# CurvineIO/curvine

Measured on AMD Instinct MI355X. Metric: cached_seq_read_GiBps, higher is better.
Workload: dtype bytes; 1 GPU; seqread; model=curvine-amd cache engine, tier=HBM, read_chunk=4194304, threads=32, iodepth=64, block_size=268435456, fuse_channels=8, short_circuit=True, parallelism=shard-per-gpu x1

## Files before the change

csrc/module.cpp:

```cpp

#include <pybind11/pybind11.h>
#include <pybind11/stl.h>

#include <sys/mman.h>

#include <atomic>
#include <cstring>
#include <mutex>
#include <stdexcept>
#include <string>
#include <vector>

#include <hip/hip_runtime.h>

namespace py = pybind11;

#define HIP_CHECK(expr)                                                        \
  do {                                                                         \
    hipError_t _e = (expr);                                                    \
    if (_e != hipSuccess)                                                      \
      throw std::runtime_error(std::string(#expr) + ": " +                     \
                               hipGetErrorString(_e));                         \
  } while (0)


static uint32_t crc_tab[8][256];
static uint32_t comb_mat[24][32];
static const uint32_t CRC_POLY = 0x82F63B78u;
static const int CRC_SUB = 4096;
static const int WG = 256;

static void gf2_square(uint32_t dst[32], const uint32_t src[32]) {
  for (int i = 0; i < 32; ++i) {
    uint32_t v = src[i], out = 0;
    for (int b = 0; b < 32; ++b)
      if ((v >> b) & 1) out ^= src[b];
    dst[i] = out;
  }
}

static uint32_t gf2_apply(const uint32_t mat[32], uint32_t crc) {
  uint32_t out = 0;
  for (int i = 0; i < 32; ++i)
    if ((crc >> i) & 1) out ^= mat[i];
  return out;
}

static void crc_init_tables() {
  for (uint32_t i = 0; i < 256; ++i) {
    uint32_t c = i;
    for (int k = 0; k < 8; ++k) c = (c >> 1) ^ ((c & 1) ? CRC_POLY : 0);
    crc_tab[0][i] = c;
  }
  for (int t = 1; t < 8; ++t)
    for (uint32_t i = 0; i < 256; ++i)
      crc_tab[t][i] = (crc_tab[t - 1][i] >> 8) ^ crc_tab[0][crc_tab[t - 1][i] & 0xFF];

  uint32_t m[32], tmp[32];
  m[0] = CRC_POLY;
  for (int i = 1; i < 32; ++i) m[i] = 1u << (i - 1);
  int shift_bits_log2 = 0;
  {
    uint64_t bits = 8ull * CRC_SUB;
    while ((1ull << shift_bits_log2) < bits) shift_bits_log2++;
  }
  for (int s = 0; s < shift_bits_log2; ++s) {
    gf2_square(tmp, m);
    std::memcpy(m, tmp, sizeof(m));
  }
  std::memcpy(comb_mat[0], m, sizeof(m));
  for (int k = 1; k < 24; ++k) gf2_square(comb_mat[k], comb_mat[k - 1]);
}

static uint32_t crc32c_sw(const uint8_t* p, size_t n, uint32_t crc_in) {
  uint32_t crc = crc_in ^ 0xFFFFFFFFu;
  while (n && ((uintptr_t)p & 7)) { crc = (crc >> 8) ^ crc_tab[0][(crc ^ *p++) & 0xFF]; --n; }
#if defined(__SSE4_2__)
  while (n >= 8) {
    crc = (uint32_t)__builtin_ia32_crc32di(crc, *(const uint64_t*)p);
    p += 8; n -= 8;
  }
  while (n) { crc = __builtin_ia32_crc32qi(crc, *p++); --n; }
#else
  while (n >= 8) {
    uint64_t v = *(const uint64_t*)p;
    uint32_t lo = (uint32_t)v ^ crc, hi = (uint32_t)(v >> 32);
    crc = crc_tab[7][lo & 0xFF] ^ crc_tab[6][(lo >> 8) & 0xFF] ^
          crc_tab[5][(lo >> 16) & 0xFF] ^ crc_tab[4][lo >> 24] ^
          crc_tab[3][hi & 0xFF] ^ crc_tab[2][(hi >> 8) & 0xFF] ^
          crc_tab[1][(hi >> 16) & 0xFF] ^ crc_tab[0][hi >> 24];
    p += 8; n -= 8;
  }
  while (n) { crc = (crc >> 8) ^ crc_tab[0][(crc ^ *p++) & 0xFF]; --n; }
#endif
  return crc ^ 0xFFFFFFFFu;
}

static uint32_t crc32c_shift(uint32_t crc, uint64_t len) {
  if (!len) return crc;
  uint32_t m[32], sq[32];
  m[0] = CRC_POLY;
  for (int i = 1; i < 32; ++i) m[i] = 1u << (i - 1);
  uint64_t bits = 8ull * len;
  while (bits) {
    if (bits & 1) crc = gf2_apply(m, crc);
    bits >>= 1;
    if (bits) { gf2_square(sq, m); std::memcpy(m, sq, sizeof(m)); }
  }
  return crc;
}

static uint32_t crc32c_combine(uint32_t crc1, uint32_t crc2, uint64_t len2) {
  return crc32c_shift(crc1, len2) ^ crc2;
}

#include "kernels.hip"
#include "lz4.hip"


static int cached_device_count = -2;
static int device_count() {
  if (cached_device_count == -2) {
    int n = 0;
    if (hipGetDeviceCount(&n) != hipSuccess) n = 0;
    cached_device_count = n;
  }
  return cached_device_count;
}


#define SPOOL 16

struct Arena {
  void* base = nullptr;
  size_t cap = 0;
  int device = -1;
  bool pinned = false;
  hipStream_t stream = nullptr;
  hipStream_t kstream = nullptr;
  hipStream_t spool[SPOOL] = {};
  std::mutex spool_mu[SPOOL];
  std::atomic<uint32_t> srr{0};
  std::vector<void*> pin;
  std::vector<hipEvent_t> ev;
  size_t pin_sz = 0;
  void* scratch = nullptr;
  size_t scratch_sz = 0;
  bool crc_tables_uploaded = false;
  bool ipc_imported = false;
  std::mutex mu;

  bool is_dev() const { return device >= 0; }
};

static std::vector<Arena*> g_arenas;
static std::mutex g_arenas_mu;

static Arena* get_arena(int h) {
  std::lock_guard<std::mutex> g(g_arenas_mu);
  if (h < 0 || h >= (int)g_arenas.size() || !g_arenas[h])
    throw std::runtime_error("bad arena handle");
  return g_arenas[h];
}

static int arena_create(int device, size_t cap, size_t staging_bytes,
                        int staging_count, bool host_pinned) {
  auto* a = new Arena();
  a->device = device;
  a->cap = cap;
  if (device >= 0) {
    if (device >= device_count()) {
      delete a;
      throw std::runtime_error("no such GPU device");
    }
    HIP_CHECK(hipSetDevice(device));
    HIP_CHECK(hipMalloc(&a->base, cap));
    HIP_CHECK(hipStreamCreateWithFlags(&a->stream, hipStreamNonBlocking));
    HIP_CHECK(hipStreamCreateWithFlags(&a->kstream, hipStreamNonBlocking));
    for (int i = 0; i < SPOOL; ++i)
      HIP_CHECK(hipStreamCreateWithFlags(&a->spool[i], hipStreamNonBlocking));
    a->pin_sz = staging_bytes;
    a->pin.resize(staging_count);
    a->ev.resize(staging_count);
    for (int i = 0; i < staging_count; ++i) {
      HIP_CHECK(hipHostMalloc(&a->pin[i], staging_bytes, hipHostMallocDefault));
      HIP_CHECK(hipEventCreateWithFlags(&a->ev[i], hipEventDisableTiming));
    }
  } else {
    if (host_pinned && device_count() > 0) {
      HIP_CHECK(hipHostMalloc(&a->base, cap, hipHostMallocDefault));
      a->pinned = true;
    } else {
      size_t aligned = (cap + ((2u << 20) - 1)) & ~size_t((2u << 20) - 1);
      if (posix_memalign(&a->base, 2u << 20, aligned) != 0) {
        delete a;
        throw std::bad_alloc();
      }
#ifdef MADV_HUGEPAGE
      madvise(a->base, aligned, MADV_HUGEPAGE);
#endif
      std::memset(a->base, 0, cap);
    }
  }
  std::lock_guard<std::mutex> g(g_arenas_mu);
  for (size_t i = 0; i < g_arenas.size(); ++i)
    if (!g_arenas[i]) { g_arenas[i] = a; return (int)i; }
  g_arenas.push_back(a);
  return (int)g_arenas.size() - 1;
}

static void arena_destroy(int h) {
  Arena* a;
  {
    std::lock_guard<std::mutex> g(g_arenas_mu);
    if (h < 0 || h >= (int)g_arenas.size() || !g_arenas[h]) return;
    a = g_arenas[h];
    g_arenas[h] = nullptr;
  }
  if (a->is_dev()) {
    hipSetDevice(a->device);
    hipStreamSynchronize(a->stream);
    for (auto* p : a->pin) hipHostFree(p);
    for (auto e : a->ev) hipEventDestroy(e);
    if (a->scratch) hipFree(a->scratch);
    if (a->ipc_imported) hipIpcCloseMemHandle(a->base);
    else hipFree(a->base);
    hipStreamDestroy(a->stream);
    hipStreamDestroy(a->kstream);
    for (int i = 0; i < SPOOL; ++i)
      if (a->spool[i]) hipStreamDestroy(a->spool[i]);
  } else if (a->pinned) {
    hipHostFree(a->base);
  } else {
    std::free(a->base);
  }
  delete a;
}


static py::bytes arena_ipc_handle(int h) {
  Arena* a = get_arena(h);
  if (!a->is_dev())
    throw std::runtime_error("ipc export: device arenas only");
  hipIpcMemHandle_t ih;
  HIP_CHECK(hipSetDevice(a->device));
  HIP_CHECK(hipIpcGetMemHandle(&ih, a->base));
  return py::bytes((const char*)&ih, sizeof(ih));
}

static int arena_ipc_open(py::bytes handle, size_t cap, int device) {
  std::string hb = handle;
  if (hb.size() != sizeof(hipIpcMemHandle_t))
    throw std::runtime_error("ipc open: bad handle size");
  if (device < 0 || device >= device_count())
    throw std::runtime_error("ipc open: bad device");
  hipIpcMemHandle_t ih;
  std::memcpy(&ih, hb.data(), sizeof(ih));
  auto* a = new Arena();
  a->device = device;
  a->cap = cap;
  a->ipc_imported = true;
  HIP_CHECK(hipSetDevice(device));
  hipError_t e = hipIpcOpenMemHandle(&a->base, ih,
                                     hipIpcMemLazyEnablePeerAccess);
  if (e != hipSuccess) {
    delete a;
    throw std::runtime_error(std::string("hipIpcOpenMemHandle: ") +
                             hipGetErrorString(e));
  }
  HIP_CHECK(hipStreamCreateWithFlags(&a->stream, hipStreamNonBlocking));
  HIP_CHECK(hipStreamCreateWithFlags(&a->kstream, hipStreamNonBlocking));
  for (int i = 0; i < SPOOL; ++i)
    HIP_CHECK(hipStreamCreateWithFlags(&a->spool[i], hipStreamNonBlocking));
  std::lock_guard<std::mutex> g(g_arenas_mu);
  for (size_t i = 0; i < g_arenas.size(); ++i)
    if (!g_arenas[i]) { g_arenas[i] = a; return (int)i; }
  g_arenas.push_back(a);
  return (int)g_arenas.size() - 1;
}

static void ensure_scratch(Arena* a, size_t n) {
  if (a->scratch_sz >= n) return;
  if (a->scratch) HIP_CHECK(hipFree(a->scratch));
  HIP_CHECK(hipMalloc(&a->scratch, n));
  a->scratch_sz = n;
}

static void ensure_crc_tables(Arena* a) {
  if (a->crc_tables_uploaded) return;
  crc_init_tables();
  HIP_CHECK(hipMemcpyToSymbol(HIP_SYMBOL(g_crc_tab), crc_tab, sizeof(crc_tab)));
  HIP_CHECK(hipMemcpyToSymbol(HIP_SYMBOL(g_comb_mat), comb_mat, sizeof(comb_mat)));
  a->crc_tables_uploaded = true;
}


static void check_range(Arena* a, uint64_t off, uint64_t n) {
  if (off + n > a->cap) throw std::runtime_error("arena range out of bounds");
}

static bool is_pinned_host(const void* p) {
  hipPointerAttribute_t at;
  if (hipPointerGetAttributes(&at, p) != hipSuccess) {
    (void)hipGetLastError();
    return false;
  }
  return at.type == hipMemoryTypeHost;
}

static const uint64_t RING_THRESHOLD = 2u << 20;


struct BouncePair {
  void* pin[2] = {nullptr, nullptr};
  hipEvent_t ev[2] = {};
  int device = -1;
};

static constexpr size_t kBounceSz = 8 << 20;

struct BouncePool {
  std::mutex mu;
  std::unordered_map<int, std::vector<BouncePair*>> free_by_dev;
};
static BouncePool g_bounce;

static BouncePair* bounce_acquire(int device) {
  {
    std::lock_guard<std::mutex> g(g_bounce.mu);
    auto& v = g_bounce.free_by_dev[device];
    if (!v.empty()) {
      BouncePair* b = v.back();
      v.pop_back();
      return b;
    }
  }
  auto* b = new BouncePair();
  b->device = device;
  HIP_CHECK(hipSetDevice(device));
  HIP_CHECK(hipHostMalloc(&b->pin[0], kBounceSz, hipHostMallocDefault));
  HIP_CHECK(hipHostMalloc(&b->pin[1], kBounceSz, hipHostMallocDefault));
  HIP_CHECK(hipEventCreateWithFlags(&b->ev[0], hipEventDisableTiming));
  HIP_CHECK(hipEventCreateWithFlags(&b->ev[1], hipEventDisableTiming));
  return b;
}

static void bounce_release(BouncePair* b) {
  std::lock_guard<std::mutex> g(g_bounce.mu);
  auto& v = g_bounce.free_by_dev[b->device];
  if (v.size() >= 32) {
    hipEventDestroy(b->ev[0]);
    hipEventDestroy(b->ev[1]);
    hipHostFree(b->pin[0]);
    hipHostFree(b->pin[1]);
    delete b;
    return;
  }
  v.push_back(b);
}

static std::atomic<bool> g_process_exiting{false};
static struct ExitFlagSetter {
  ~ExitFlagSetter() { g_process_exiting.store(true); }
} g_exit_flag_setter;

struct TlsStreams {
  hipStream_t s[64] = {};
  ~TlsStreams() {
    if (g_process_exiting.load()) return;
    for (auto x : s)
      if (x) (void)hipStreamDestroy(x);
  }
};

static hipStream_t thread_stream(int device) {
  thread_local TlsStreams tls;
  if (device < 0 || device >= 64) throw std::runtime_error("bad device");
  if (!tls.s[device]) {
    HIP_CHECK(hipSetDevice(device));
    HIP_CHECK(hipStreamCreateWithFlags(&tls.s[device], hipStreamNonBlocking));
  }
  return tls.s[device];
}

static void dev_read_direct(Arena* a, uint64_t off, uint8_t* dst, uint64_t n) {
  HIP_CHECK(hipSetDevice(a->device));
  hipStream_t s = thread_stream(a->device);
  HIP_CHECK(hipMemcpyAsync(dst, (const uint8_t*)a->base + off, n,
                           hipMemcpyDeviceToHost, s));
  HIP_CHECK(hipStreamSynchronize(s));
}

static void dev_write_direct(Arena* a, uint64_t off, const uint8_t* src,
                             uint64_t n) {
  HIP_CHECK(hipSetDevice(a->device));
  hipStream_t s = thread_stream(a->device);
  HIP_CHECK(hipMemcpyAsync((uint8_t*)a->base + off, src, n,
                           hipMemcpyHostToDevice, s));
  HIP_CHECK(hipStreamSynchronize(s));
}

static void dev_read(Arena* a, uint64_t off, uint8_t* dst, uint64_t n) {
  if (n <= RING_THRESHOLD || is_pinned_host(dst)) {
    dev_read_direct(a, off, dst, n);
    return;
  }
  HIP_CHECK(hipSetDevice(a->device));
  BouncePair* bp = bounce_acquire(a->device);
  hipStream_t s = thread_stream(a->device);
  const uint8_t* src = (const uint8_t*)a->base + off;
  uint64_t cs = std::min<uint64_t>(kBounceSz,
                                   std::max<uint64_t>(1u << 20, (n + 1) / 2));
  uint64_t nchunks = (n + cs - 1) / cs;
  try {
    for (uint64_t c = 0; c < nchunks; ++c) {
      uint64_t coff = c * cs;
      uint64_t clen = std::min<uint64_t>(cs, n - coff);
      int slot = (int)(c & 1);
      HIP_CHECK(hipMemcpyAsync(bp->pin[slot], src + coff, clen,
                               hipMemcpyDeviceToHost, s));
      HIP_CHECK(hipEventRecord(bp->ev[slot], s));
      if (c > 0) {
        int prev = (int)((c - 1) & 1);
        HIP_CHECK(hipEventSynchronize(bp->ev[prev]));
        uint64_t poff = (c - 1) * cs;
        std::memcpy(dst + poff, bp->pin[prev],
                    std::min<uint64_t>(cs, n - poff));
      }
    }
    int last = (int)((nchunks - 1) & 1);
    HIP_CHECK(hipEventSynchronize(bp->ev[last]));
    uint64_t loff = (nchunks - 1) * cs;
    std::memcpy(dst + loff, bp->pin[last],
                std::min<uint64_t>(cs, n - loff));
  } catch (...) {
    (void)hipStreamSynchronize(s);
    bounce_release(bp);
    throw;
  }
  bounce_release(bp);
}

static void dev_write(Arena* a, uint64_t off, const uint8_t* src, uint64_t n) {
  if (n <= RING_THRESHOLD || is_pinned_host(src)) {
    dev_write_direct(a, off, src, n);
    return;
  }
  HIP_CHECK(hipSetDevice(a->device));
  BouncePair* bp = bounce_acquire(a->device);
  hipStream_t s = thread_stream(a->device);
  uint8_t* dst = (uint8_t*)a->base + off;
  uint64_t cs = std::min<uint64_t>(kBounceSz,
                                   std::max<uint64_t>(1u << 20, (n + 1) / 2));
  uint64_t nchunks = (n + cs - 1) / cs;
  try {
    for (uint64_t c = 0; c < nchunks; ++c) {
      uint64_t coff = c * cs;
      uint64_t clen = std::min<uint64_t>(cs, n - coff);
      int slot = (int)(c & 1);
      if (c >= 2) HIP_CHECK(hipEventSynchronize(bp->ev[slot]));
      std::memcpy(bp->pin[slot], src + coff, clen);
      HIP_CHECK(hipMemcpyAsync(dst + coff, bp->pin[slot], clen,
                               hipMemcpyHostToDevice, s));
// ... 262 lines not shown
        uint64_t doff = d2 * a->pin_sz;
        std::memcpy(dst + doff, a->pin[ds],
                    std::min<uint64_t>(a->pin_sz, total - doff));
      }
    }
  }
}

static void arena_gather_ptr(
    int h, std::vector<std::tuple<uint64_t, uint64_t, uint64_t>> ext,
    uintptr_t dst_ptr) {
  Arena* a = get_arena(h);
  for (auto& e : ext) check_range(a, std::get<0>(e), std::get<2>(e));
  uint8_t* dst = (uint8_t*)dst_ptr;
  py::gil_scoped_release rel;
  if (!a->is_dev()) {
    for (auto& e : ext)
      std::memcpy(dst + std::get<1>(e), (uint8_t*)a->base + std::get<0>(e),
                  std::get<2>(e));
    return;
  }
  std::lock_guard<std::mutex> g(a->mu);
  HIP_CHECK(hipSetDevice(a->device));
  std::vector<Extent> exts(ext.size());
  std::vector<uint32_t> tile_ext;
  std::vector<uint64_t> tile_off;
  for (size_t i = 0; i < ext.size(); ++i) {
    exts[i] = {std::get<0>(ext[i]), std::get<1>(ext[i]), std::get<2>(ext[i])};
    for (uint64_t t = 0; t < exts[i].len; t += TILE) {
      tile_ext.push_back((uint32_t)i);
      tile_off.push_back(t);
    }
  }
  size_t meta = exts.size() * sizeof(Extent) +
                tile_ext.size() * (sizeof(uint32_t) + sizeof(uint64_t)) + 64;
  ensure_scratch(a, meta);
  Extent* d_ext = (Extent*)a->scratch;
  uint32_t* d_te = (uint32_t*)(d_ext + exts.size());
  uint64_t* d_to = (uint64_t*)(((uintptr_t)(d_te + tile_ext.size()) + 7) & ~7ull);
  HIP_CHECK(hipMemcpyAsync(d_ext, exts.data(), exts.size() * sizeof(Extent),
                           hipMemcpyHostToDevice, a->kstream));
  HIP_CHECK(hipMemcpyAsync(d_te, tile_ext.data(),
                           tile_ext.size() * sizeof(uint32_t),
                           hipMemcpyHostToDevice, a->kstream));
  HIP_CHECK(hipMemcpyAsync(d_to, tile_off.data(),
                           tile_off.size() * sizeof(uint64_t),
                           hipMemcpyHostToDevice, a->kstream));
  int grid = (int)std::min<size_t>(tile_ext.size(), 8192);
  (void)hipGetLastError();
  hipLaunchKernelGGL(copy_extents_kernel, dim3(grid), dim3(WG), 0, a->kstream,
                     (const uint8_t*)a->base, dst, d_ext, d_te, d_to,
                     (uint32_t)tile_ext.size());
  HIP_CHECK(hipGetLastError());
  HIP_CHECK(hipStreamSynchronize(a->kstream));
}

static uintptr_t arena_base_ptr(int h) {
  return (uintptr_t)get_arena(h)->base;
}

static void arena_read_batch(int h, const std::vector<uint64_t>& offs,
                             const std::vector<uint64_t>& dsts, uint64_t n) {
  Arena* a = get_arena(h);
  if (offs.size() != dsts.size())
    throw std::runtime_error("arena_read_batch: offs/dsts mismatch");
  for (uint64_t off : offs) check_range(a, off, n);
  py::gil_scoped_release rel;
  if (!a->is_dev()) {
    for (size_t i = 0; i < offs.size(); ++i)
      std::memcpy((uint8_t*)dsts[i], (uint8_t*)a->base + offs[i], n);
    return;
  }
  HIP_CHECK(hipSetDevice(a->device));
  hipStream_t s = thread_stream(a->device);
  for (size_t i = 0; i < offs.size(); ++i)
    HIP_CHECK(hipMemcpyAsync((void*)dsts[i], (uint8_t*)a->base + offs[i], n,
                             hipMemcpyDeviceToHost, s));
  HIP_CHECK(hipStreamSynchronize(s));
}


struct RdExt { uint64_t file_off, len; int arena; uint64_t arena_off; };
struct RdReader { uint64_t length; std::vector<RdExt> exts; };
static std::mutex g_rd_mu;
static std::unordered_map<int64_t, RdReader> g_rd;
static int64_t g_rd_next = 1;

static int64_t reader_register(
    std::vector<std::tuple<uint64_t, uint64_t, int, uint64_t>> exts,
    uint64_t length) {
  RdReader r;
  r.length = length;
  r.exts.reserve(exts.size());
  uint64_t prev = 0;
  for (auto& e : exts) {
    if (std::get<0>(e) < prev)
      throw std::runtime_error("reader_register: extents must be sorted");
    prev = std::get<0>(e);
    get_arena(std::get<2>(e));
    r.exts.push_back({std::get<0>(e), std::get<1>(e), std::get<2>(e),
                      std::get<3>(e)});
  }
  std::lock_guard<std::mutex> g(g_rd_mu);
  int64_t rid = g_rd_next++;
  g_rd[rid] = std::move(r);
  return rid;
}

static void reader_unregister(int64_t rid) {
  std::lock_guard<std::mutex> g(g_rd_mu);
  g_rd.erase(rid);
}

static py::list reader_pread_batch(int64_t rid,
                                   const std::vector<uint64_t>& offs,
                                   uint64_t n, uintptr_t dst_ptr,
                                   uint64_t stride) {
  RdReader* r;
  {
    std::lock_guard<std::mutex> g(g_rd_mu);
    auto it = g_rd.find(rid);
    if (it == g_rd.end()) throw std::runtime_error("bad reader id");
    r = &it->second;
  }
  std::vector<uint32_t> skipped;
  {
    py::gil_scoped_release rel;
    int used_dev[8];
    int n_dev = 0;
    const auto& exts = r->exts;
    for (size_t i = 0; i < offs.size(); ++i) {
      uint64_t off = offs[i];
      const RdExt* e = nullptr;
      if (off + n <= r->length && !exts.empty()) {
        size_t lo = 0, hi = exts.size();
        while (lo < hi) {
          size_t mid = (lo + hi) / 2;
          if (exts[mid].file_off <= off) lo = mid + 1; else hi = mid;
        }
        if (lo > 0 && off - exts[lo - 1].file_off + n <= exts[lo - 1].len)
          e = &exts[lo - 1];
      }
      if (e == nullptr) {
        skipped.push_back((uint32_t)i);
        continue;
      }
      uint64_t boff = off - e->file_off;
      Arena* a = get_arena(e->arena);
      uint8_t* dst = (uint8_t*)dst_ptr + i * stride;
      const uint8_t* src = (uint8_t*)a->base + e->arena_off + boff;
      if (!a->is_dev()) {
        std::memcpy(dst, src, n);
      } else {
        HIP_CHECK(hipSetDevice(a->device));
        HIP_CHECK(hipMemcpyAsync(dst, src, n, hipMemcpyDeviceToHost,
                                 thread_stream(a->device)));
        bool seen = false;
        for (int d = 0; d < n_dev; d++) seen |= (used_dev[d] == a->device);
        if (!seen && n_dev < 8) used_dev[n_dev++] = a->device;
      }
    }
    for (int d = 0; d < n_dev; d++) {
      HIP_CHECK(hipSetDevice(used_dev[d]));
      HIP_CHECK(hipStreamSynchronize(thread_stream(used_dev[d])));
    }
  }
  py::list out;
  for (uint32_t i : skipped) out.append(i);
  return out;
}


static py::bytes lz4_compress_py(py::buffer buf) {
  py::buffer_info info = buf.request(false);
  const uint8_t* src = (const uint8_t*)info.ptr;
  size_t n = (size_t)info.size * info.itemsize;
  uint32_t n_chunks = (uint32_t)((n + LZ4_CHUNK - 1) / LZ4_CHUNK);
  std::vector<uint32_t> sizes(n_chunks);
  std::vector<uint8_t> out;
  out.reserve(n / 2 + 1024);
  size_t header = 4 + 8 + 4 + 4 + 4ull * n_chunks;
  out.resize(header);
  {
    py::gil_scoped_release rel;
    std::vector<uint8_t> tmp(LZ4_CHUNK + LZ4_CHUNK / 128 + 64);
    for (uint32_t c = 0; c < n_chunks; ++c) {
      size_t cn = std::min<size_t>(LZ4_CHUNK, n - (size_t)c * LZ4_CHUNK);
      size_t cs = lz4_compress_block(src + (size_t)c * LZ4_CHUNK, cn,
                                     tmp.data());
      sizes[c] = (uint32_t)cs;
      out.insert(out.end(), tmp.data(), tmp.data() + cs);
    }
    uint8_t* h = out.data();
    memcpy(h, &LZ4_MAGIC, 4);
    uint64_t raw = n;
    memcpy(h + 4, &raw, 8);
    uint32_t ck = LZ4_CHUNK;
    memcpy(h + 12, &ck, 4);
    memcpy(h + 16, &n_chunks, 4);
    memcpy(h + 20, sizes.data(), 4ull * n_chunks);
  }
  return py::bytes((const char*)out.data(), out.size());
}

struct Lz4Header {
  uint64_t raw_size;
  uint32_t chunk_size, n_chunks;
  const uint32_t* sizes;
  const uint8_t* payload;
};

static Lz4Header lz4_parse(const uint8_t* p, size_t n) {
  if (n < 20) throw std::runtime_error("lz4: short container");
  uint32_t magic;
  memcpy(&magic, p, 4);
  if (magic != LZ4_MAGIC) throw std::runtime_error("lz4: bad magic");
  Lz4Header h;
  memcpy(&h.raw_size, p + 4, 8);
  memcpy(&h.chunk_size, p + 12, 4);
  memcpy(&h.n_chunks, p + 16, 4);
  if (n < 20 + 4ull * h.n_chunks) throw std::runtime_error("lz4: truncated");
  h.sizes = (const uint32_t*)(p + 20);
  h.payload = p + 20 + 4ull * h.n_chunks;
  uint64_t payload_n = 0;
  for (uint32_t c = 0; c < h.n_chunks; ++c) payload_n += h.sizes[c];
  if (payload_n > n - 20 - 4ull * h.n_chunks)
    throw std::runtime_error("lz4: truncated");
  if ((uint64_t)h.n_chunks * h.chunk_size < h.raw_size ||
      (h.n_chunks && (uint64_t)(h.n_chunks - 1) * h.chunk_size >= h.raw_size))
    throw std::runtime_error("lz4: chunk table does not match raw size");
  return h;
}

static py::bytes lz4_decompress_py(py::buffer buf) {
  py::buffer_info info = buf.request(false);
  const uint8_t* src = (const uint8_t*)info.ptr;
  size_t n = (size_t)info.size * info.itemsize;
  Lz4Header h = lz4_parse(src, n);
  std::string out(h.raw_size, '\0');
  {
    py::gil_scoped_release rel;
    const uint8_t* p = h.payload;
    for (uint32_t c = 0; c < h.n_chunks; ++c) {
      size_t cap = std::min<uint64_t>(h.chunk_size,
                                      h.raw_size - (uint64_t)c * h.chunk_size);
      size_t got = lz4_decompress_block_host(
          p, h.sizes[c], (uint8_t*)out.data() + (uint64_t)c * h.chunk_size,
          cap);
      if (got != cap) throw std::runtime_error("lz4: corrupt chunk");
      p += h.sizes[c];
    }
  }
// ... 136 lines not shown
                               tile_off.size() * sizeof(uint64_t),
                               hipMemcpyHostToDevice, a->kstream));
      hipLaunchKernelGGL(copy_extents_kernel,
                         dim3((int)std::min<size_t>(tile_ext.size(), 8192)),
                         dim3(WG), 0, a->kstream, (const uint8_t*)d_slots,
                         d_pack, d_ext, d_te, d_to, (uint32_t)tile_ext.size());
      HIP_CHECK(hipGetLastError());
      out.resize(header + total);
      HIP_CHECK(hipMemcpyAsync(out.data() + header, d_pack, total,
                               hipMemcpyDeviceToHost, a->kstream));
      HIP_CHECK(hipStreamSynchronize(a->kstream));
    }
    uint8_t* h = out.data();
    memcpy(h, &LZ4_MAGIC, 4);
    memcpy(h + 4, &n, 8);
    uint32_t ck = LZ4_CHUNK;
    memcpy(h + 12, &ck, 4);
    memcpy(h + 16, &n_chunks, 4);
    memcpy(h + 20, sizes.data(), 4ull * n_chunks);
  }
  return py::bytes((const char*)out.data(), out.size());
}


extern "C" {
typedef struct { int32_t device_type; int32_t device_id; } DLDevice;
typedef struct { uint8_t code; uint8_t bits; uint16_t lanes; } DLDataType;
typedef struct {
  void* data; DLDevice device; int32_t ndim; DLDataType dtype;
  int64_t* shape; int64_t* strides; uint64_t byte_offset;
} DLTensor;
typedef struct DLManagedTensor {
  DLTensor dl_tensor; void* manager_ctx;
  void (*deleter)(struct DLManagedTensor*);
} DLManagedTensor;
}
static const int kDLCPU = 1, kDLROCM = 10;

struct DLWrap { DLManagedTensor mt; int64_t shape[1]; };

static void dl_deleter(DLManagedTensor* mt) {
  delete reinterpret_cast<DLWrap*>(mt->manager_ctx);
}

static void dl_capsule_destructor(PyObject* cap) {
  if (PyCapsule_IsValid(cap, "dltensor")) {
    auto* mt = (DLManagedTensor*)PyCapsule_GetPointer(cap, "dltensor");
    if (mt && mt->deleter) mt->deleter(mt);
  }
}

static py::object arena_dlpack(int h, uint64_t off, uint64_t n) {
  Arena* a = get_arena(h);
  check_range(a, off, n);
  auto* w = new DLWrap();
  w->shape[0] = (int64_t)n;
  w->mt.dl_tensor.data = (uint8_t*)a->base + off;
  w->mt.dl_tensor.device = {a->is_dev() ? kDLROCM : kDLCPU,
                            a->is_dev() ? a->device : 0};
  w->mt.dl_tensor.ndim = 1;
  w->mt.dl_tensor.dtype = {0 , 8, 1};
  w->mt.dl_tensor.dtype.code = 1;
  w->mt.dl_tensor.shape = w->shape;
  w->mt.dl_tensor.strides = nullptr;
  w->mt.dl_tensor.byte_offset = 0;
  w->mt.manager_ctx = w;
  w->mt.deleter = dl_deleter;
  PyObject* cap = PyCapsule_New(&w->mt, "dltensor", dl_capsule_destructor);
  return py::reinterpret_steal<py::object>(cap);
}

static py::memoryview arena_host_view(int h, uint64_t off, uint64_t n) {
  Arena* a = get_arena(h);
  if (a->is_dev()) throw std::runtime_error("arena_host_view: device arena");
  check_range(a, off, n);
  return py::memoryview::from_memory((uint8_t*)a->base + off, n, false);
}


struct PinnedBuf { void* ptr = nullptr; size_t n = 0; bool pinned = false; };
static std::vector<PinnedBuf> g_pins;
static std::mutex g_pins_mu;

static int pinned_alloc(size_t n) {
  PinnedBuf b;
  b.n = n;
  if (device_count() > 0) {
    HIP_CHECK(hipHostMalloc(&b.ptr, n, hipHostMallocDefault));
    b.pinned = true;
  } else {
    b.ptr = std::malloc(n);
    if (!b.ptr) throw std::bad_alloc();
  }
  std::lock_guard<std::mutex> g(g_pins_mu);
  for (size_t i = 0; i < g_pins.size(); ++i)
    if (!g_pins[i].ptr) { g_pins[i] = b; return (int)i; }
  g_pins.push_back(b);
  return (int)g_pins.size() - 1;
}

static void pinned_free(int id) {
  std::lock_guard<std::mutex> g(g_pins_mu);
  if (id < 0 || id >= (int)g_pins.size() || !g_pins[id].ptr) return;
  if (g_pins[id].pinned) hipHostFree(g_pins[id].ptr);
  else std::free(g_pins[id].ptr);
  g_pins[id] = PinnedBuf{};
}

static py::memoryview pinned_view(int id) {
  std::lock_guard<std::mutex> g(g_pins_mu);
  if (id < 0 || id >= (int)g_pins.size() || !g_pins[id].ptr)
    throw std::runtime_error("bad pinned buffer id");
  return py::memoryview::from_memory(g_pins[id].ptr, g_pins[id].n, false);
}

static uintptr_t pinned_ptr(int id) {
  std::lock_guard<std::mutex> g(g_pins_mu);
  if (id < 0 || id >= (int)g_pins.size() || !g_pins[id].ptr)
    throw std::runtime_error("bad pinned buffer id");
  return (uintptr_t)g_pins[id].ptr;
}

static py::dict arena_info(int h) {
  Arena* a = get_arena(h);
  py::dict d;
  d["capacity"] = a->cap;
  d["device"] = a->device;
  d["pinned"] = a->pinned;
  d["staging_bytes"] = a->pin_sz;
  d["staging_count"] = a->pin.size();
  return d;
}

static void memcpy_h2d(uintptr_t dst, uintptr_t src, uint64_t n) {
  py::gil_scoped_release rel;
  HIP_CHECK(hipMemcpy((void*)dst, (const void*)src, n, hipMemcpyHostToDevice));
}

static void device_sync(int device) {
  py::gil_scoped_release rel;
  HIP_CHECK(hipSetDevice(device));
  HIP_CHECK(hipDeviceSynchronize());
}

#include "fuse_loop.hip"

#include "meta_server.cpp"
#include "data_server.cpp"
#include "sdk_abi.cpp"

static py::dict device_mem_info(int device) {
  size_t free_b = 0, total_b = 0;
  HIP_CHECK(hipSetDevice(device));
  HIP_CHECK(hipMemGetInfo(&free_b, &total_b));
  py::dict d;
  d["free"] = free_b;
  d["total"] = total_b;
  return d;
}

PYBIND11_MODULE(_native, m) {
  m.doc() = "curvine_amd native data plane (HIP/CDNA4, gfx950)";
  m.def("device_count", &device_count);
  m.def("device_sync", &device_sync);
  m.def("memcpy_h2d", &memcpy_h2d);
  m.def("device_mem_info", &device_mem_info);
  m.def("arena_ipc_handle", &arena_ipc_handle);
  m.def("arena_ipc_open", &arena_ipc_open);
  m.def("arena_create", &arena_create, py::arg("device"), py::arg("capacity"),
        py::arg("staging_bytes") = 4 << 20, py::arg("staging_count") = 8,
        py::arg("host_pinned") = false);
  m.def("arena_destroy", &arena_destroy);
  m.def("arena_read", &arena_read);
  m.def("arena_write", &arena_write);
  m.def("arena_read_ptr", &arena_read_ptr);
  m.def("arena_write_ptr", &arena_write_ptr);
  m.def("arena_copy", &arena_copy);
  m.def("arena_fill", &arena_fill);
  m.def("arena_crc32c", &arena_crc32c);
  m.def("arena_gather", &arena_gather);
  m.def("arena_gather_ptr", &arena_gather_ptr);
  m.def("arena_base_ptr", &arena_base_ptr);
  m.def("arena_read_batch", &arena_read_batch);
  m.def("reader_register", &reader_register);
  m.def("reader_unregister", &reader_unregister);
  m.def("reader_pread_batch", &reader_pread_batch);
  m.def("arena_info", &arena_info);
  m.def("arena_dlpack", &arena_dlpack);
  m.def("arena_host_view", &arena_host_view);
  m.def("pinned_alloc", &pinned_alloc);
  m.def("pinned_free", &pinned_free);
  m.def("pinned_view", &pinned_view);
  m.def("pinned_ptr", &pinned_ptr);
  m.def("fuse_loop_create", &fuse_loop_create);
  m.def("fuse_loop_add_channel", &fuse_loop_add_channel);
  m.def("fuse_loop_register", &fuse_loop_register);
  m.def("fuse_loop_unregister", &fuse_loop_unregister);
  m.def("fuse_loop_register_write", &fuse_loop_register_write);
  m.def("fuse_loop_unregister_write", &fuse_loop_unregister_write);
  m.def("fuse_loop_write_state", &fuse_loop_write_state);
  m.def("fuse_loop_next_forward", &fuse_loop_next_forward);
  m.def("fuse_loop_stats", &fuse_loop_stats);
  m.def("fuse_loop_stop", &fuse_loop_stop);
  m.def("meta_create", &meta_create);
  m.def("meta_stop", &meta_stop_srv);
  m.def("meta_set_serving", &meta_set_serving);
  m.def("meta_upsert", &meta_upsert);
  m.def("meta_upsert_node", &meta_upsert_node);
  m.def("meta_touch", &meta_touch);
  m.def("meta_upsert_with_children", &meta_upsert_with_children);
  m.def("meta_add_child", &meta_add_child);
  m.def("meta_remove_child", &meta_remove_child);
  m.def("meta_drop", &meta_drop);
  m.def("meta_clear", &meta_clear);
  m.def("meta_forward_pop", &meta_forward_pop);
  m.def("meta_eventfd", &meta_eventfd);
  m.def("meta_send", &meta_send);
  m.def("meta_stats", &meta_stats);
  m.def("meta_worker_upsert", &meta_worker_upsert);
  m.def("meta_block_add_loc", &meta_block_add_loc);
  m.def("meta_block_remove_loc", &meta_block_remove_loc);
  m.def("meta_block_drop", &meta_block_drop);
  m.def("meta_take_access", &meta_take_access);
  m.def("data_create", &data_create);
  m.def("data_stop", &data_stop_srv);
  m.def("data_block_publish", &data_block_publish, py::arg("sid"),
        py::arg("block_id"), py::arg("kind"), py::arg("arena"),
        py::arg("aoff"), py::arg("len"), py::arg("path"),
        py::arg("direct") = false);
  m.def("data_block_drop", &data_block_drop);
  m.def("data_block_refs", &data_block_refs);
  m.def("data_write_register", &data_write_register);
  m.def("data_write_unregister", &data_write_unregister);
  m.def("data_forward_pop", &data_forward_pop);
  m.def("data_eventfd", &data_eventfd);
  m.def("data_send", &data_send);
  m.def("data_stats", &data_stats);
  m.def("data_read_into", &data_read_into);
  m.def("data_write_from", &data_write_from);
  m.def("dw_open", &dw_open);
  m.def("dw_write", &dw_write);
  m.def("dw_drain", &dw_drain);
  m.def("dw_commit", &dw_commit);
  m.def("dw_abort", &dw_abort);
  m.def("lz4_compress", &lz4_compress_py);
  m.def("lz4_decompress", &lz4_decompress_py);
  m.def("arena_lz4_decompress", &arena_lz4_decompress);
  m.def("arena_lz4_compress", &arena_lz4_compress);
  m.def("crc32c", &crc32c_buf, py::arg("buf"), py::arg("init") = 0);
  m.def("crc32c_combine", &crc32c_combine);
  m.attr("CRC_SUB") = CRC_SUB;
  m.attr("__hip_arch__") = "gfx950";
}
```

curvine_amd/client/reader.py:

```python
from __future__ import annotations

import asyncio

from curvine_amd import errors as err
from curvine_amd.client.block_client import (BlockReaderHole, BlockReaderLocal,
                                             BlockReaderRemote)
from curvine_amd.client.fs_client import FsClient
from curvine_amd.model import FileBlocks, LocatedBlock


class ReadDetector:

    def __init__(self):
        self.last_end = 0
        self.seq_count = 0
        self.rand_count = 0

    def observe(self, off: int, n: int) -> None:
        if off == self.last_end:
            self.seq_count += 1
        else:
            self.rand_count += 1
        self.last_end = off + n

    @property
    def is_sequential(self) -> bool:
        return self.seq_count >= self.rand_count



def _hole_span(offs, blocks, length, pos) -> int:
    import bisect
    idx = bisect.bisect_right(offs, pos) - 1
    nxt = idx + 1
    if idx >= 0:
        lb = blocks[idx]
        if pos < lb.offset + lb.block.length:
            return 0
    end = offs[nxt] if nxt < len(offs) else length
    return max(0, end - pos)


class SyncLocalReader:

    def __init__(self, file_blocks: FileBlocks, ipc_resolver=None):
        from curvine_amd.worker import registry
        self.fb = file_blocks
        self.length = file_blocks.status.length
        self._offs = [b.offset for b in file_blocks.blocks]
        self._readers = []
        self._native_rid = None
        try:
            for lb in file_blocks.blocks:
                r = None
                for addr in lb.locations:
                    store = registry.lookup(addr.worker_id)
                    if store is not None:
                        r = store.open_reader(lb.block.block_id)
                        break
                if r is None and ipc_resolver is not None:
                    r = ipc_resolver(lb)
                if r is None:
                    raise err.BlockNotFound(
                        f"block {lb.block.block_id} has no in-process replica")
                self._readers.append(r)
        except Exception:
            self.close()
            raise
        self._try_register_native()

    def _try_register_native(self) -> None:
        exts = []
        for lb, r in zip(self.fb.blocks, self._readers):
            meta = r.meta
            arena = getattr(r.layout, "arena", None)
            if meta.get("kind") != "arena" or arena is None:
                return
            exts.append((lb.offset, lb.block.length, arena.handle,
                         meta["offset"]))
        if not exts:
            return
        try:
            from curvine_amd import native
            self._native_rid = native.load().reader_register(
                exts, self.length)
        except Exception:
            self._native_rid = None

    def pread_into(self, off: int, out, out_off: int, n: int) -> int:
        import bisect
        n = max(0, min(n, self.length - off))
        got = 0
        while got < n:
            pos = off + got
            hole = _hole_span(self._offs, self.fb.blocks, self.length, pos)
            if hole > 0:
                fill = min(hole, n - got)
                out[out_off + got:out_off + got + fill] = b"\x00" * fill
                got += fill
                continue
            idx = bisect.bisect_right(self._offs, pos) - 1
            if idx < 0 or idx >= len(self._readers):
                break
            lb = self.fb.blocks[idx]
            boff = pos - lb.offset
            want = min(n - got, lb.block.length - boff)
            got += self._readers[idx].read_into(boff, out, out_off + got, want)
        return got

    def pread_into_ptr(self, off: int, ptr: int, n: int) -> int:
        import bisect
        import ctypes
        n = max(0, min(n, self.length - off))
        got = 0
        while got < n:
            pos = off + got
            hole = _hole_span(self._offs, self.fb.blocks, self.length, pos)
            if hole > 0:
                fill = min(hole, n - got)
                ctypes.memset(ptr + got, 0, fill)
                got += fill
                continue
            idx = bisect.bisect_right(self._offs, pos) - 1
            if idx < 0 or idx >= len(self._readers):
                break
            lb = self.fb.blocks[idx]
            boff = pos - lb.offset
            want = min(n - got, lb.block.length - boff)
            got += self._readers[idx].read_to_ptr(boff, ptr + got, want, False)
        return got

    def pread(self, off: int, n: int) -> bytes:
        out = bytearray(max(0, min(n, self.length - off)))
        got = self.pread_into(off, out, 0, len(out))
        return bytes(out[:got])

    def pread_batch_ptr(self, file_offs: list[int], n: int, dst_ptr: int,
                        stride: int) -> int:
        import bisect
        import ctypes
        from curvine_amd import native
        if not self.fb.blocks:
            return 0
        if self._native_rid is not None:
            skipped = native.load().reader_pread_batch(
                self._native_rid, file_offs, n, dst_ptr, stride)
            for i in skipped:
                buf = bytearray(n)
                got = self.pread_into(file_offs[i], buf, 0, n)
                ctypes.memmove(dst_ptr + i * stride, bytes(buf[:got]), got)
            return len(file_offs)
        groups: dict[int, tuple[list, list]] = {}
        slow: list[tuple[int, int]] = []
        for i, off in enumerate(file_offs):
            idx = max(0, bisect.bisect_right(self._offs, off) - 1)
            lb = self.fb.blocks[idx]
            boff = off - lb.offset
            r = self._readers[idx]
            meta = r.meta
            if meta.get("kind") == "arena" and boff + n <= lb.block.length:
                offs, dsts = groups.setdefault(r.layout.arena.handle, ([], []))
                offs.append(meta["offset"] + boff)
                dsts.append(dst_ptr + i * stride)
            else:
                slow.append((i, off))
        mod = native.load()
        for h, (offs, dsts) in groups.items():
            mod.arena_read_batch(h, offs, dsts, n)
        for i, off in slow:
            buf = bytearray(n)
            got = self.pread_into(off, buf, 0, n)
            ctypes.memmove(dst_ptr + i * stride, bytes(buf[:got]), got)
        return len(file_offs)

    def pread_gather(self, samples: list[tuple[int, int, int]],
                     dst_ptr: int, dst_on_device: bool = False) -> int:
        groups, slow, total = self.resolve_gather(samples, dst_on_device)
        self.exec_gather(groups, slow, dst_ptr)
        return total

    def resolve_gather(self, samples, dst_on_device: bool):
        import bisect
        groups: dict[int, tuple[object, list]] = {}
        slow: list[tuple[int, int, int]] = []
        total = 0
        for off, n, doff in samples:
            n = max(0, min(n, self.length - off))
            got = 0
            while got < n:
                idx = bisect.bisect_right(self._offs, off + got) - 1
                lb = self.fb.blocks[idx]
                boff = off + got - lb.offset
                want = min(n - got, lb.block.length - boff)
                if want <= 0:
                    break
# ... 277 lines not shown
```

curvine_amd/native.py:

```python
from __future__ import annotations

import os
import subprocess
import sys
import sysconfig
import threading

_REPO = os.path.dirname(os.path.dirname(os.path.abspath(__file__)))
_SO = os.path.join(_REPO, "curvine_amd", "_native.so")
_SRC = os.path.join(_REPO, "csrc", "module.cpp")
_SRC2 = os.path.join(_REPO, "csrc", "kernels.hip")
_SRC3 = os.path.join(_REPO, "csrc", "lz4.hip")
_SRC4 = os.path.join(_REPO, "csrc", "fuse_loop.hip")
_SRC5 = os.path.join(_REPO, "csrc", "meta_server.cpp")
_SRC6 = os.path.join(_REPO, "csrc", "data_server.cpp")
_SRC7 = os.path.join(_REPO, "csrc", "sdk_abi.cpp")
_lock = threading.Lock()
_mod = None


def build_native(force: bool = False) -> str:
    if not force and os.path.exists(_SO) and os.path.exists(_SRC):
        if os.path.getmtime(_SO) >= max(os.path.getmtime(_SRC),
                                        os.path.getmtime(_SRC2),
# ... 74 lines not shown
        out = bytearray(n)
        self._n.arena_read(self.handle, off, out, 0, n)
        return bytes(out)

    def read_to_ptr(self, off: int, dst_ptr: int, n: int, device: bool) -> None:
        self._n.arena_read_ptr(self.handle, off, dst_ptr, n, device)

    def write_from_ptr(self, off: int, src_ptr: int, n: int, device: bool) -> None:
        self._n.arena_write_ptr(self.handle, off, src_ptr, n, device)

    def copy_to(self, dst: "Arena", dst_off: int, src_off: int, n: int) -> None:
        self._n.arena_copy(dst.handle, dst_off, self.handle, src_off, n)

    def fill(self, off: int, n: int, value: int = 0) -> None:
        self._n.arena_fill(self.handle, off, n, value)

    def crc32c(self, off: int, n: int) -> int:
        return self._n.arena_crc32c(self.handle, off, n)

    def gather(self, extents: list[tuple[int, int]], out, out_off: int = 0) -> None:
        self._n.arena_gather(self.handle, extents, out, out_off)

    def gather_ptr(self, triples: list[tuple[int, int, int]],
                   dst_ptr: int) -> None:
        self._n.arena_gather_ptr(self.handle, triples, dst_ptr)

    def lz4_compress(self, off: int, n: int) -> bytes:
        return self._n.arena_lz4_compress(self.handle, off, n)

    def lz4_decompress_into(self, off: int, container) -> int:
        return self._n.arena_lz4_decompress(self.handle, off, container)

    def base_ptr(self) -> int:
        return self._n.arena_base_ptr(self.handle)

    def ipc_handle(self) -> bytes:
        return self._n.arena_ipc_handle(self.handle)

    @classmethod
    def from_ipc(cls, handle: bytes, capacity: int, device: int) -> "Arena":
        self = cls.__new__(cls)
        self._n = load()
        self.device = device
        self.capacity = capacity
        self.handle = self._n.arena_ipc_open(handle, capacity, device)
        self._closed = False
        return self

    def close(self) -> None:
        if not self._closed:
            self._n.arena_destroy(self.handle)
            self._closed = True

    def __del__(self):
        try:
            self.close()
        except Exception:
            pass


class PinnedBuffer:

    def __init__(self, nbytes: int):
        self._n = load()
        self.nbytes = nbytes
        self.id = self._n.pinned_alloc(nbytes)
        self.view = self._n.pinned_view(self.id)
        self.ptr = self._n.pinned_ptr(self.id)
        self._closed = False

    def close(self) -> None:
        if not self._closed:
            self.view = None
            self._n.pinned_free(self.id)
            self._closed = True

    def __del__(self):
        try:
            self.close()
        except Exception:
            pass


def crc32c(buf, init: int = 0) -> int:
    return load().crc32c(buf, init)


def crc32c_combine(crc1: int, crc2: int, len2: int) -> int:
    return load().crc32c_combine(crc1, crc2, len2)


def lz4_compress(buf) -> bytes:
    return load().lz4_compress(buf)


def lz4_decompress(buf) -> bytes:
    return load().lz4_decompress(buf)
```

Measured before the change: 47.79 GiB/s.

## Add native pread_into_ptr path, pinned/stream pools, and shared-lock registries

Adds a native reader_pread_ptr that resolves extents and issues device-to-host copies in C++ with the GIL released, so the Python bisect and ctypes loop is skipped on the read path. It also pools pinned host buffers and per-thread HIP streams to avoid repeated hipHostMalloc and stream creation, and switches the arena and reader registries to shared_mutex with shared_ptr readers to cut lock contention among the 32 reader threads. Stats counters and a trim function are added. The risks are pooled pinned memory being held longer than before and a stream taken from the pool needing a synchronize before reuse.

New measurement: 49.22 GiB/s, median of 4. +3.0%, better.

```diff
diff --git a/csrc/module.cpp b/csrc/module.cpp
--- a/csrc/module.cpp
+++ b/csrc/module.cpp
@@ -6,9 +6,12 @@
 
 #include <atomic>
 #include <cstring>
+#include <memory>
 #include <mutex>
+#include <shared_mutex>
 #include <stdexcept>
 #include <string>
+#include <unordered_map>
 #include <vector>
 
 #include <hip/hip_runtime.h>
@@ -153,11 +156,18 @@
   bool is_dev() const { return device >= 0; }
 };
 
+static std::atomic<uint64_t> g_st_pinned_real_allocs{0};
+static std::atomic<uint64_t> g_st_pinned_pool_hits{0};
+static std::atomic<uint64_t> g_st_streams_created{0};
+static std::atomic<uint64_t> g_st_streams_reused{0};
+static std::atomic<uint64_t> g_st_pread_ptr_native{0};
+static std::atomic<uint64_t> g_st_pread_ptr_fallback{0};
+
 static std::vector<Arena*> g_arenas;
-static std::mutex g_arenas_mu;
+static std::shared_mutex g_arenas_mu;
 
 static Arena* get_arena(int h) {
-  std::lock_guard<std::mutex> g(g_arenas_mu);
+  std::shared_lock<std::shared_mutex> g(g_arenas_mu);
   if (h < 0 || h >= (int)g_arenas.size() || !g_arenas[h])
     throw std::runtime_error("bad arena handle");
   return g_arenas[h];
@@ -202,7 +212,7 @@
       std::memset(a->base, 0, cap);
     }
   }
-  std::lock_guard<std::mutex> g(g_arenas_mu);
+  std::unique_lock<std::shared_mutex> g(g_arenas_mu);
   for (size_t i = 0; i < g_arenas.size(); ++i)
     if (!g_arenas[i]) { g_arenas[i] = a; return (int)i; }
   g_arenas.push_back(a);
@@ -212,7 +222,7 @@
 static void arena_destroy(int h) {
   Arena* a;
   {
-    std::lock_guard<std::mutex> g(g_arenas_mu);
+    std::unique_lock<std::shared_mutex> g(g_arenas_mu);
     if (h < 0 || h >= (int)g_arenas.size() || !g_arenas[h]) return;
     a = g_arenas[h];
     g_arenas[h] = nullptr;
@@ -272,7 +282,7 @@
   HIP_CHECK(hipStreamCreateWithFlags(&a->kstream, hipStreamNonBlocking));
   for (int i = 0; i < SPOOL; ++i)
     HIP_CHECK(hipStreamCreateWithFlags(&a->spool[i], hipStreamNonBlocking));
-  std::lock_guard<std::mutex> g(g_arenas_mu);
+  std::unique_lock<std::shared_mutex> g(g_arenas_mu);
   for (size_t i = 0; i < g_arenas.size(); ++i)
     if (!g_arenas[i]) { g_arenas[i] = a; return (int)i; }
   g_arenas.push_back(a);
@@ -364,21 +374,61 @@
   ~ExitFlagSetter() { g_process_exiting.store(true); }
 } g_exit_flag_setter;
 
+static constexpr int kMaxDevices = 64;
+static constexpr size_t kStreamPoolMax = 64;
+
+struct StreamPool {
+  std::mutex mu;
+  std::vector<hipStream_t> free_by_dev[kMaxDevices];
+};
+static StreamPool& stream_pool() {
+  static StreamPool* p = new StreamPool();
+  return *p;
+}
+
 struct TlsStreams {
-  hipStream_t s[64] = {};
+  hipStream_t s[kMaxDevices] = {};
   ~TlsStreams() {
     if (g_process_exiting.load()) return;
-    for (auto x : s)
-      if (x) (void)hipStreamDestroy(x);
+    for (int d = 0; d < kMaxDevices; ++d) {
+      hipStream_t x = s[d];
+      if (!x) continue;
+      {
+        StreamPool& sp = stream_pool();
+        std::lock_guard<std::mutex> g(sp.mu);
+        if (sp.free_by_dev[d].size() < kStreamPoolMax) {
+          sp.free_by_dev[d].push_back(x);
+          continue;
+        }
+      }
+      (void)hipStreamDestroy(x);
+    }
   }
 };
 
 static hipStream_t thread_stream(int device) {
   thread_local TlsStreams tls;
-  if (device < 0 || device >= 64) throw std::runtime_error("bad device");
+  if (device < 0 || device >= kMaxDevices)
+    throw std::runtime_error("bad device");
   if (!tls.s[device]) {
-    HIP_CHECK(hipSetDevice(device));
-    HIP_CHECK(hipStreamCreateWithFlags(&tls.s[device], hipStreamNonBlocking));
+    {
+      StreamPool& sp = stream_pool();
+      std::lock_guard<std::mutex> g(sp.mu);
+      auto& v = sp.free_by_dev[device];
+      if (!v.empty()) {
+        tls.s[device] = v.back();
+        v.pop_back();
+      }
+    }
+    if (tls.s[device]) {
+      HIP_CHECK(hipStreamSynchronize(tls.s[device]));
+      g_st_streams_reused.fetch_add(1, std::memory_order_relaxed);
+    } else {
+      HIP_CHECK(hipSetDevice(device));
+      HIP_CHECK(hipStreamCreateWithFlags(&tls.s[device],
+                                         hipStreamNonBlocking));
+      g_st_streams_created.fetch_add(1, std::memory_order_relaxed);
+    }
   }
   return tls.s[device];
 }
@@ -807,9 +857,26 @@
 
 struct RdExt { uint64_t file_off, len; int arena; uint64_t arena_off; };
 struct RdReader { uint64_t length; std::vector<RdExt> exts; };
-static std::mutex g_rd_mu;
-static std::unordered_map<int64_t, RdReader> g_rd;
+static std::shared_mutex g_rd_mu;
+static std::unordered_map<int64_t, std::shared_ptr<const RdReader>> g_rd;
 static int64_t g_rd_next = 1;
+
+static std::shared_ptr<const RdReader> rd_lookup(int64_t rid) {
+  std::shared_lock<std::shared_mutex> g(g_rd_mu);
+  auto it = g_rd.find(rid);
+  if (it == g_rd.end()) throw std::runtime_error("bad reader id");
+  return it->second;
+}
+
+static const RdExt* rd_floor_ext(const RdReader& r, uint64_t off) {
+  const auto& exts = r.exts;
+  size_t lo = 0, hi = exts.size();
+  while (lo < hi) {
+    size_t mid = (lo + hi) / 2;
+    if (exts[mid].file_off <= off) lo = mid + 1; else hi = mid;
+  }
+  return lo > 0 ? &exts[lo - 1] : nullptr;
+}
 
 static int64_t reader_register(
     std::vector<std::tuple<uint64_t, uint64_t, int, uint64_t>> exts,
@@ -826,14 +893,14 @@
     r.exts.push_back({std::get<0>(e), std::get<1>(e), std::get<2>(e),
                       std::get<3>(e)});
   }
-  std::lock_guard<std::mutex> g(g_rd_mu);
+  std::unique_lock<std::shared_mutex> g(g_rd_mu);
   int64_t rid = g_rd_next++;
-  g_rd[rid] = std::move(r);
+  g_rd[rid] = std::make_shared<const RdReader>(std::move(r));
   return rid;
 }
 
 static void reader_unregister(int64_t rid) {
-  std::lock_guard<std::mutex> g(g_rd_mu);
+  std::unique_lock<std::shared_mutex> g(g_rd_mu);
   g_rd.erase(rid);
 }
 
@@ -841,30 +908,18 @@
                                    const std::vector<uint64_t>& offs,
                                    uint64_t n, uintptr_t dst_ptr,
                                    uint64_t stride) {
-  RdReader* r;
-  {
-    std::lock_guard<std::mutex> g(g_rd_mu);
-    auto it = g_rd.find(rid);
-    if (it == g_rd.end()) throw std::runtime_error("bad reader id");
-    r = &it->second;
-  }
+  std::shared_ptr<const RdReader> r = rd_lookup(rid);
   std::vector<uint32_t> skipped;
   {
     py::gil_scoped_release rel;
     int used_dev[8];
     int n_dev = 0;
-    const auto& exts = r->exts;
     for (size_t i = 0; i < offs.size(); ++i) {
       uint64_t off = offs[i];
       const RdExt* e = nullptr;
-      if (off + n <= r->length && !exts.empty()) {
-        size_t lo = 0, hi = exts.size();
-        while (lo < hi) {
-          size_t mid = (lo + hi) / 2;
-          if (exts[mid].file_off <= off) lo = mid + 1; else hi = mid;
-        }
-        if (lo > 0 && off - exts[lo - 1].file_off + n <= exts[lo - 1].len)
-          e = &exts[lo - 1];
+      if (off + n <= r->length) {
+        e = rd_floor_ext(*r, off);
+        if (e && off - e->file_off + n > e->len) e = nullptr;
       }
       if (e == nullptr) {
         skipped.push_back((uint32_t)i);
@@ -893,6 +948,75 @@
   py::list out;
   for (uint32_t i : skipped) out.append(i);
   return out;
+}
+
+static int64_t reader_pread_ptr(int64_t rid, uint64_t off, uint64_t n,
+                                uintptr_t dst_ptr) {
+  std::shared_ptr<const RdReader> r = rd_lookup(rid);
+  if (off >= r->length) n = 0;
+  else n = std::min<uint64_t>(n, r->length - off);
+  struct Piece { Arena* a; const uint8_t* src; uint64_t dst_off, len; };
+  Piece inl[4];
+  std::vector<Piece> spill;
+  size_t n_pieces = 0;
+  for (uint64_t got = 0; got < n;) {
+    uint64_t pos = off + got;
+    const RdExt* e = rd_floor_ext(*r, pos);
+    if (e == nullptr || pos - e->file_off >= e->len) {
+      g_st_pread_ptr_fallback.fetch_add(1, std::memory_order_relaxed);
+      return -1;
+    }
+    uint64_t boff = pos - e->file_off;
+    uint64_t want = std::min<uint64_t>(n - got, e->len - boff);
+    Arena* a = get_arena(e->arena);
+    check_range(a, e->arena_off + boff, want);
+    Piece p{a, (const uint8_t*)a->base + e->arena_off + boff, got, want};
+    if (n_pieces < 4) {
+      inl[n_pieces] = p;
+    } else {
+      if (spill.empty()) spill.assign(inl, inl + 4);
+      spill.push_back(p);
+    }
+    ++n_pieces;
+    got += want;
+  }
+  const Piece* pieces = spill.empty() ? inl : spill.data();
+  int used_dev[8];
+  int n_dev = 0;
+  auto sync_used = [&](bool check) {
+    for (int d = 0; d < n_dev; d++) {
+      hipError_t e1 = hipSetDevice(used_dev[d]);
+      hipError_t e2 = e1 == hipSuccess
+          ? hipStreamSynchronize(thread_stream(used_dev[d])) : e1;
+      if (check) HIP_CHECK(e2);
+    }
+  };
+  try {
+    for (size_t i = 0; i < n_pieces; ++i) {
+      const Piece& p = pieces[i];
+      uint8_t* dst = (uint8_t*)dst_ptr + p.dst_off;
+      if (!p.a->is_dev()) {
+        std::memcpy(dst, p.src, p.len);
+        continue;
+      }
+      bool seen = false;
+      for (int d = 0; d < n_dev; d++) seen |= (used_dev[d] == p.a->device);
+      if (!seen && n_dev == 8) {
+        sync_used(true);
+        n_dev = 0;
+      }
+      HIP_CHECK(hipSetDevice(p.a->device));
+      hipStream_t s = thread_stream(p.a->device);
+      if (!seen) used_dev[n_dev++] = p.a->device;
+      HIP_CHECK(hipMemcpyAsync(dst, p.src, p.len, hipMemcpyDeviceToHost, s));
+    }
+    sync_used(true);
+  } catch (...) {
+    sync_used(false);
+    throw;
+  }
+  g_st_pread_ptr_native.fetch_add(1, std::memory_order_relaxed);
+  return (int64_t)n;
 }
 
 
@@ -1195,11 +1319,29 @@
 static std::vector<PinnedBuf> g_pins;
 static std::mutex g_pins_mu;
 
+static constexpr size_t kPinnedPoolMaxBytes = 8 * 2 * kBounceSz;
+static std::unordered_map<size_t, std::vector<void*>> g_pin_free;
+static size_t g_pin_free_bytes = 0;
+
 static int pinned_alloc(size_t n) {
   PinnedBuf b;
   b.n = n;
   if (device_count() > 0) {
-    HIP_CHECK(hipHostMalloc(&b.ptr, n, hipHostMallocDefault));
+    {
+      std::lock_guard<std::mutex> g(g_pins_mu);
+      auto it = g_pin_free.find(n);
+      if (it != g_pin_free.end() && !it->second.empty()) {
+        b.ptr = it->second.back();
+        it->second.pop_back();
+        g_pin_free_bytes -= n;
+      }
+    }
+    if (b.ptr) {
+      g_st_pinned_pool_hits.fetch_add(1, std::memory_order_relaxed);
+    } else {
+      HIP_CHECK(hipHostMalloc(&b.ptr, n, hipHostMallocDefault));
+      g_st_pinned_real_allocs.fetch_add(1, std::memory_order_relaxed);
+    }
     b.pinned = true;
   } else {
     b.ptr = std::malloc(n);
@@ -1213,11 +1355,50 @@
 }
 
 static void pinned_free(int id) {
-  std::lock_guard<std::mutex> g(g_pins_mu);
-  if (id < 0 || id >= (int)g_pins.size() || !g_pins[id].ptr) return;
-  if (g_pins[id].pinned) hipHostFree(g_pins[id].ptr);
-  else std::free(g_pins[id].ptr);
-  g_pins[id] = PinnedBuf{};
+  PinnedBuf b;
+  {
+    std::lock_guard<std::mutex> g(g_pins_mu);
+    if (id < 0 || id >= (int)g_pins.size() || !g_pins[id].ptr) return;
+    b = g_pins[id];
+    g_pins[id] = PinnedBuf{};
+    if (b.pinned && b.n <= kPinnedPoolMaxBytes - g_pin_free_bytes) {
+      g_pin_free[b.n].push_back(b.ptr);
+      g_pin_free_bytes += b.n;
+      return;
+    }
+  }
+  if (b.pinned) hipHostFree(b.ptr);
+  else std::free(b.ptr);
+}
+
+static size_t pinned_pool_trim() {
+  std::unordered_map<size_t, std::vector<void*>> drop;
+  size_t bytes;
+  {
+    std::lock_guard<std::mutex> g(g_pins_mu);
+    drop.swap(g_pin_free);
+    bytes = g_pin_free_bytes;
+    g_pin_free_bytes = 0;
+  }
+  for (auto& kv : drop)
+    for (void* p : kv.second) hipHostFree(p);
+  return bytes;
+}
+
+static py::dict native_stats() {
+  py::dict d;
+  d["pinned_real_allocs"] = g_st_pinned_real_allocs.load();
+  d["pinned_pool_hits"] = g_st_pinned_pool_hits.load();
+  d["streams_created"] = g_st_streams_created.load();
+  d["streams_reused"] = g_st_streams_reused.load();
+  d["pread_ptr_native"] = g_st_pread_ptr_native.load();
+  d["pread_ptr_fallback"] = g_st_pread_ptr_fallback.load();
+  {
+    std::lock_guard<std::mutex> g(g_pins_mu);
+    d["pinned_pool_bytes"] = g_pin_free_bytes;
+  }
+  d["pinned_pool_max_bytes"] = kPinnedPoolMaxBytes;
+  return d;
 }
 
 static py::memoryview pinned_view(int id) {
@@ -1298,6 +1479,10 @@
   m.def("reader_register", &reader_register);
   m.def("reader_unregister", &reader_unregister);
   m.def("reader_pread_batch", &reader_pread_batch);
+  m.def("reader_pread_ptr", &reader_pread_ptr,
+        py::call_guard<py::gil_scoped_release>());
+  m.def("native_stats", &native_stats);
+  m.def("pinned_pool_trim", &pinned_pool_trim);
   m.def("arena_info", &arena_info);
   m.def("arena_dlpack", &arena_dlpack);
   m.def("arena_host_view", &arena_host_view);
diff --git a/curvine_amd/client/reader.py b/curvine_amd/client/reader.py
--- a/curvine_amd/client/reader.py
+++ b/curvine_amd/client/reader.py
@@ -82,8 +82,9 @@
             return
         try:
             from curvine_amd import native
-            self._native_rid = native.load().reader_register(
-                exts, self.length)
+            mod = native.load()
+            self._native_pread_ptr = mod.reader_pread_ptr
+            self._native_rid = mod.reader_register(exts, self.length)
         except Exception:
             self._native_rid = None
 
@@ -111,6 +112,10 @@
     def pread_into_ptr(self, off: int, ptr: int, n: int) -> int:
         import bisect
         import ctypes
+        if self._native_rid is not None and off >= 0 and n >= 0:
+            got = self._native_pread_ptr(self._native_rid, off, n, ptr)
+            if got >= 0:
+                return got
         n = max(0, min(n, self.length - off))
         got = 0
         while got < n:
diff --git a/curvine_amd/native.py b/curvine_amd/native.py
--- a/curvine_amd/native.py
+++ b/curvine_amd/native.py
@@ -180,6 +180,10 @@
             pass
 
 
+def pinned_pool_trim() -> int:
+    return load().pinned_pool_trim()
+
+
 def crc32c(buf, init: int = 0) -> int:
     return load().crc32c(buf, init)
 
```
